# heracles-ec/heracles

Hardware: AMD Instinct MI355X
Metric: map->Cl pairs/sec + mixing-matrix build sec, nside=4096 lmax=6144 (higher is better)
Workload: dtype f64

## Files before the change

### heracles_amd/csrc/hx_analysis.hip

```cpp
#include <algorithm>
#include <cmath>
#include <cstdlib>
#include <cstring>

#include "hx_sht_common.h"

namespace hx {
using namespace hxfft;

constexpr int HALF_F = 1;
template <int SPIN>
struct LegCfg {
    static constexpr int NW = SPIN == 0 ? 16 : 8;
    static constexpr int NT = SPIN == 0 ? 1 : 2;
    static constexpr int NOP = SPIN == 0 ? 1 : 2;
    static constexpr int NPAR = (SPIN == 2 && HALF_F) ? 1 : 2;
};
int analysis_f_rows(int spin) { return spin == 0 ? LegCfg<0>::NPAR * LegCfg<0>::NOP : LegCfg<2>::NPAR * LegCfg<2>::NOP; }

struct LegParams {
    PlanDev P;
    const LegTask *__restrict__ tasks;
    const double *__restrict__ F;
    double *__restrict__ partial;
// ... 510 lines not shown
        if (l >= l0) {
            const int col = (c >> 3) * NCOL + 2 * (c & 7);
            for (int t = 0; t < mt.count; ++t) {
                const double *p = partial + (tasks[mt.first + t].pout - row0 + (l - l0)) * ncol + col;
                v.x += p[0];
                v.y += p[1];
            }
            if (fl) { v.x *= fl[l]; v.y *= fl[l]; }
        }
        double2 *dst = alm + (long long)c * alm_stride + almidx(lmax, l, m);
        if (add) { const double2 o = *dst; v.x += o.x; v.y += o.y; }
        *dst = v;
    }
}

static int ring_mlim(int lmax, int spin, double sth, double cth)
{
    double ofs = lmax * 0.01;
    if (ofs < 100.) ofs = 100.;
    double b = -2 * spin * fabs(cth);
    double t1 = lmax * sth + ofs;
    double c = (double)spin * spin - t1 * t1;
    double discr = b * b - 4 * c;
    if (discr <= 0) return lmax;
    double res = (-b + sqrt(discr)) / 2.;
    if (res > lmax) res = lmax;
    return (int)(res + 0.5);
}

struct SweepShape {
    int ng, nbx, valu, ncol, oneset, duo;
};
static SweepShape sweep_shape(int spin, int nb)
{
    const int cols = 2 * nb;
    SweepShape sh = {0, 0, 0, 0, 0, 0};
    if (cols <= 8) { sh.valu = 1; return sh; }
    sh.duo = 1;
    sh.oneset = spin == 2;
    sh.ng = std::max(cols / NCOL, 1);
    const int rem = cols > NCOL ? cols % NCOL : 0;
    const int maxbx = spin == 2 ? 2 : (sh.ng == 1 ? 1 : 0);
    if (rem > 4 * maxbx) sh.ng += 1;
// ... 147 lines not shown
    hx_plan::TaskSet &ts = blocks == 8 && blocks != valu_task_blocks(spin) ? (spin ? pl->ts[6] : pl->ts[7]) : (spin ? pl->ts[4] : pl->ts[5]);
    HX_TRY(build_task_set(pl, spin, blocks, ts));
    *out = &ts;
    return HX_OK;
}

int synth_duo_tasks(hx_plan *pl, int spin, hx_plan::TaskSet **out)
{
    if (spin) HX_TRY(ensure_rec2(pl));
    hx_plan::TaskSet &ts = spin ? pl->ts[3] : pl->ts[2];
    HX_TRY(build_task_set(pl, spin, PipeCfg<2>::NW * (spin ? PipeCfg<2>::RBS : PipeCfg<0>::RBS), ts));
    DevBuf &lim = spin ? pl->syn_mlim2 : pl->syn_mlim0;
    if (!lim.p) {
        std::vector<int> h(pl->nrp_pad, -1);
        for (int rp = 0; rp < pl->nrp; ++rp) {
            const int last = std::min(rp / RBLK * RBLK + RBLK - 1, pl->nrp - 1);
            h[rp] = std::min(pl->lmax, ring_mlim(pl->lmax, spin, pl->h_sth[last], pl->h_z[last]));
        }
        HX_TRY(upload(lim, h));
    }
    *out = &ts;
    return HX_OK;
}

static int analysis_batch_valu(hx_plan *pl, int spin, int nb, const double *d_maps, double2 *d_alms, const double *d_rw,
                               const double *d_pw, const double *d_fl, int add)
{
    hx_plan::TaskSet *tsp = nullptr;
    HX_TRY(valu_tasks(pl, spin, &tsp));
    hx_plan::TaskSet &ts = *tsp;
    if (pl->hsrc == nullptr && pl->nssrc == nullptr) {
        HX_TRY(pl->Y.alloc(sizeof(double2) * (size_t)pl->ny * nb));
        HX_TRY(launch_ring_subdft_maps(pl, nb, d_maps, d_pw, pl->Y.as<double2>()));
    }
    double budget = 80e9;
    if (scratch_budget_bytes() > 0.0) budget = scratch_budget_bytes();
    else {
        size_t fr = 0, tot = 0;
        if (hipMemGetInfo(&fr, &tot) == hipSuccess) budget = std::min(budget, 0.5 * (double)(fr + pl->F.bytes + pl->partial.bytes));
        budget = std::max(budget, 2e9);
    }
    const int lmax = pl->lmax, pcol = valu_partial_cols(spin), unit = spin ? 2 : 1;
    const double f_per_m = (double)pl->nrp_pad * valu_operand_doubles(spin) * sizeof(double);
    const std::vector<long long> &prow = ts.rows_before_m;
    std::vector<std::pair<int, int>> chunks;
    size_t maxF = 16, maxP = 16;
    const int m_end = pl->m_hi < 0 ? lmax + 1 : std::min(pl->m_hi, lmax + 1), ms = std::max(pl->m_step, 1);
    for (int m0 = std::max(pl->m_lo, 0); m0 < m_end;) {
// ... 31 lines not shown

int analysis_batch(hx_plan *pl, int spin, int nb, const double *d_maps, double2 *d_alms, const double *d_rw,
                   const double *d_pw, const double *d_fl, int add)
{
    if (valu_batch(spin, nb)) return analysis_batch_valu(pl, spin, nb, d_maps, d_alms, d_rw, d_pw, d_fl, add);
    const int sidx = spin ? 1 : 0;
    HX_TRY(build_tasks(pl, spin));
    if (spin) HX_TRY(ensure_rec2(pl));
    const SweepShape sh = sweep_shape(spin, nb);
    const bool one_set = sh.oneset || duo_shape(sh);
    if (one_set) HX_TRY(build_task_set(pl, spin, PipeCfg<2>::NW * (spin ? PipeCfg<2>::RBS : PipeCfg<0>::RBS), spin ? pl->ts[3] : pl->ts[2]));
    hx_plan::TaskSet &ts = one_set ? (spin ? pl->ts[3] : pl->ts[2]) : pl->ts[sidx];
    const int ncol = sh.ncol;
    if (pl->hsrc == nullptr && pl->nssrc == nullptr) {
        HX_TRY(pl->Y.alloc(sizeof(double2) * (size_t)pl->ny * nb));
        HX_TRY(launch_ring_subdft_maps(pl, nb, d_maps, d_pw, pl->Y.as<double2>()));
    }

    double budget = 80e9;
    if (scratch_budget_bytes() > 0.0) budget = scratch_budget_bytes();
    else {
        size_t fr = 0, tot = 0;
        if (hipMemGetInfo(&fr, &tot) == hipSuccess)
            budget = std::min(budget, 0.5 * (double)(fr + pl->F.bytes + pl->partial.bytes));
        budget = std::max(budget, 2e9);
    }
    const double f_per_m = (double)pl->nrp_pad * analysis_f_rows(spin) * ncol * sizeof(double);
    const int lmax = pl->lmax;
    const std::vector<long long> &prow = ts.arow;
    const int pcol = sweep_pcol(sh);
    std::vector<std::pair<int, int>> chunks;
// ... 99 lines not shown
    HX_HIP(hipMemsetAsync(pl->partial.p, 0, (size_t)stream_tasks(pl, s.spin).arow[pl->lmax + 1] * sweep_pcol(sh) * sizeof(double), rt().stream));
    pl->last_chunks = 1;
    return HX_OK;
}

template <int SPIN>
static int stream_slab(StreamSweep &s, int k)
{
    hx_plan *pl = s.pl;
    hx_plan::TaskSet &ts = stream_tasks(pl, SPIN);
    const SweepShape sh = sweep_shape(SPIN, s.nb);
    const int ng = sh.ng + (sh.nbx > 0 ? 1 : 0), lmax = pl->lmax, nm = lmax + 1;
    const int rp_lo = s.rp_edge[k], rp_hi = s.rp_edge[k + 1];
    hipStream_t st = rt().stream;
    PlanDev P = pl->dev();
    HX_TRY(launch_ring_subdft_maps(pl, s.nb, s.d_maps, s.d_pw, pl->Y.as<double2>(), rp_lo, std::min(rp_hi, pl->nrp)));
    {
        ProfScope ps("fourier_combine");
        const int tile_hi = k + 1 == s.nslab ? pl->nrp_pad / 32 : rp_hi / 32;
        dim3 grid(nm, tile_hi - rp_lo / 32);
        hipLaunchKernelGGL(k_fourier_combine<SPIN>, grid, dim3(256), 0, st, P, pl->Y.as<double2>(), s.nb, ng, sh.ncol, 0, 1, s.d_rw,
                           ts.d_tasks.as<LegTask>(), ts.d_of_m.as<MTasks>(), pl->F.as<double>(), rp_lo / 32);
    }
    {
        ProfScope ps("legendre_analysis");
        ProfScope ps2(SPIN == 0 ? "legendre_analysis_s0" : "legendre_analysis_s2");
        LegParams A;
        A.P = P; A.tasks = ts.d_tasks.as<LegTask>(); A.F = pl->F.as<double>(); A.partial = pl->partial.as<double>();
        A.m0 = 0; A.ms = 1; A.row0 = 0; A.ng = ng; A.ncol = sh.ncol; A.pcol = sweep_pcol(sh);
        A.of_m = s.d_of_m.as<MTasks>() + (size_t)k * (lmax + 1); A.arow = ts.d_arow.as<long long>(); A.arow0 = 0; A.add_all = 1;
        HX_TRY(launch_duo<SPIN>(sh, dim3((unsigned)nm), st, A, SPIN == 0 ? pl->cn0.as<double2>() : pl->cn2.as<double2>()));
// ... 90 lines not shown
```

### heracles_amd/csrc/hx_fft_core.h

```cpp
#pragma once
#ifdef __HIPCC__
#include <hip/hip_runtime.h>
#define HX_HD __host__ __device__ __forceinline__
#else
#include <cmath>
#define HX_HD inline
struct double2 {
    double x, y;
};
#endif

namespace hxfft {

HX_HD double2 mk(double a, double b)
{
    double2 r;
    r.x = a;
    r.y = b;
    return r;
}
HX_HD double2 cadd(double2 a, double2 b) { return mk(a.x + b.x, a.y + b.y); }
HX_HD double2 csub(double2 a, double2 b) { return mk(a.x - b.x, a.y - b.y); }
HX_HD double2 cmul(double2 a, double2 b) { return mk(a.x * b.x - a.y * b.y, a.x * b.y + a.y * b.x); }
HX_HD double2 cmulc(double2 a, double2 b)
// ... 16 lines not shown
}

HX_HD int ilog2(unsigned v)
{
    int p = 0;
    while ((1u << p) < v) ++p;
    return p;
}

HX_HD int fft_size_for(int n)
{
    if ((n & (n - 1)) == 0) return n;
    int m = 1;
    while (m < 2 * n - 1) m <<= 1;
    return m;
}

struct TwFactored {
    const double2 *hi, *lo;
    HX_HD double2 operator[](int k) const
    {
        const double2 a = hi[k >> 6], b = lo[k & 63];
        double2 r;
        r.x = a.x * b.x - a.y * b.y;
        r.y = a.x * b.y + a.y * b.x;
        return r;
    }
};

HX_HD int lds_slot(int e) { return e + (e >> 4) + (e >> 9); }
// ... 159 lines not shown
```

### heracles_amd/csrc/hx_legendre_valu.hip

```cpp
#include <algorithm>
#include <cmath>

#include "hx_sht_common.h"

namespace hx {
using namespace hxfft;

constexpr int VALU_R0 = 8;
constexpr int VALU_R2 = 6;
constexpr int VALU_LB0 = 8;
constexpr int VALU_LB2 = 4;
template <int SPIN>
struct ValuCfg {
    static constexpr int R = SPIN == 0 ? VALU_R0 : VALU_R2;
    static constexpr int LB = SPIN == 0 ? VALU_LB0 : VALU_LB2;
    static constexpr int NA = SPIN == 0 ? 2 : 4;
    static constexpr int NF = SPIN == 0 ? 4 : 8;
    static constexpr int NRB = 2 * R;
    static_assert(LB * NA == 32 || LB * NA == 16, "the butterfly below reduces 16 or 32 accumulators");
};

int valu_task_blocks(int spin) { return spin == 0 ? ValuCfg<0>::NRB : ValuCfg<2>::NRB; }
int valu_partial_cols(int spin) { return spin == 0 ? ValuCfg<0>::NA : ValuCfg<2>::NA; }
int valu_operand_doubles(int spin) { return spin == 0 ? ValuCfg<0>::NF : ValuCfg<2>::NF; }
// ... 5 lines not shown
    const LegTask *__restrict__ tasks;
    const double *__restrict__ F;
    double *__restrict__ partial;
    int m0, ms;
    long long row0;
};

template <int SPIN>
__global__ __launch_bounds__(256) void k_fourier_combine_valu(PlanDev P, const double2 *__restrict__ Y, int c0, int m0, int ms,
                                                              const double *__restrict__ rw, const LegTask *__restrict__ tasks,
                                                              const MTasks *__restrict__ of_m, double *__restrict__ F)
{
    constexpr int NF = ValuCfg<SPIN>::NF;
    const int m = m0 + blockIdx.x * ms;
    const MTasks mt = of_m[m];
    if (mt.count == 0 || ((int)blockIdx.y + 1) * 256 <= tasks[mt.first].rb0 * RBLK) return;
    const int rp = blockIdx.y * 256 + threadIdx.x;
    if (rp >= P.nrp_pad) return;
    double *row = F + ((long long)blockIdx.x * P.nrp_pad + rp) * NF;
    double o[NF];
#pragma unroll
    for (int k = 0; k < NF; ++k) o[k] = 0.0;
    if (rp < P.nrp) {
        const RingAtM ram = ring_at_m_of(P, rp, m, rw);
        if (SPIN == 0) {
            double2 fn, fs;
            ring_modes_ns(P, Y, c0, rp, m, ram, fn, fs);
            o[0] = fn.x + fs.x; o[1] = fn.y + fs.y;
            o[2] = fn.x - fs.x; o[3] = fn.y - fs.y;
        } else {
            double2 qn, qs, un, us;
            ring_modes_ns(P, Y, c0, rp, m, ram, qn, qs);
// ... 626 lines not shown
```

### heracles_amd/csrc/hx_sht.hip

```cpp
#include <algorithm>
#include <chrono>
#include <cmath>
#include <cstdlib>

#include <type_traits>

#include "hx_sht_common.h"


namespace hx {
using namespace hxfft;

__global__ void k_init_norm0(int lmax, double2 *__restrict__ coef, double *__restrict__ alpha)
{
    const int t = blockIdx.x * blockDim.x + threadIdx.x;
    const int m = t >> 1, par = t & 1;
    if (m > lmax) return;
    const double dm = m;
    auto a = [dm](double l) { return sqrt((4.0 * l * l - 1.0) / (l * l - dm * dm)); };
    double al = 1.0;
    for (int l = m + par; l <= lmax; l += 2) {
        const double dl = l;
        const double a1 = a(dl + 1.0), a2 = a(dl + 2.0);
        const double A = a1 * a2;
// ... 23 lines not shown
        const double r1 = sqrt((2.0 * k + 3.0) / (2.0 * k + 1.0));
        const double p = r1 * (2.0 * k + 1.0) * k * lp / den;
        const double q = -r1 * (2.0 * k + 1.0) * dm * dn / den;
        double a1 = 1.0;
        if (l > l0) {
            const double r2 = sqrt((2.0 * k + 3.0) / (2.0 * k - 1.0));
            const double r = r2 * lp * sqrt((k * k - dm * dm) * (k * k - dn * dn)) / den;
            a1 = r * am1;
        }
        coef[almidx(lmax, l + 1, m)] = make_double2(p * a0 / a1, q * a0 / a1);
        am1 = a0;
        a0 = a1;
    }
}

__global__ __launch_bounds__(512) void k_init_bhat(PlanDev P, const int *__restrict__ rp_list,
                                                   double2 *__restrict__ bhat)
{
    extern __shared__ double2 buf[];
    const int rp = rp_list[blockIdx.x];
    const int n = P.nsub[rp];
    const int M = fft_size_for(n);
    for (int j = threadIdx.x; j < lds_fft_slots(M); j += blockDim.x) buf[j] = make_double2(0.0, 0.0);
    __syncthreads();
    for (int j = threadIdx.x; j < n; j += blockDim.x) {
        double2 c = expipi((double)chirp_num(j, n) / (double)n);
        buf[lds_slot(j)] = c;
        if (j) buf[lds_slot(M - j)] = c;
    }
    __syncthreads();
    lds_fft_dif(buf, M, P.tw, P.twN);
    double2 *out = bhat + P.bhat_off[rp];
    for (int e = threadIdx.x; e < M; e += blockDim.x) out[M >= 16 ? (e & 15) * (M >> 4) + (e >> 4) : e] = buf[lds_slot(e)];
}

__host__ __device__ inline int ring_ph_hi(int M) { return (4 * M) / 64 + 1; }
constexpr int RING_NTMAX = 512;
constexpr int RING_FB = 8;

template <int MODE, bool WSYM = false>
__global__ __launch_bounds__(RING_NTMAX) void k_ring_subdft(PlanDev P, const RingDesc *__restrict__ desc, int nrings, int nb, int Mclass,
                                                            const double *__restrict__ maps,
                                                            const double *__restrict__ pixw,
                                                            const double2 *__restrict__ zin,
                                                            double2 *__restrict__ Y, double *__restrict__ pixout = nullptr,
                                                            const double *__restrict__ ref = nullptr)
{
// ... 6 lines not shown
    int tid = threadIdx.x;
    auto ring_of = [&](int item) __attribute__((always_inline)) { return ((item >> 5) / nb) * 8 + (item & 7); };
    RingDesc cur = RingDesc{0, 0, 0, 1, 0};
    if ((int)blockIdx.x < nitems && ring_of(blockIdx.x) < nrings) cur = desc[ring_of(blockIdx.x)];
    for (int item = blockIdx.x; item < nitems; item += gridDim.x) {
        const int r = (item >> 3) & 3, set = item >> 5;
        const int ring = ring_of(item), c = set % nb;
        const int itn = item + gridDim.x, ringn = itn < nitems ? ring_of(itn) : nrings;
        const bool nextv = ringn < nrings;
        if (ring >= nrings) {
            if (nextv) cur = desc[ringn];
            continue;
        }
        const int n = cur.n;
        const long long sN = cur.sN, sS = cur.sS;
        const int M = fft_size_for(n), MP = lds_fft_slots(M);
        const bool blu = M != n;
        const int p = ilog2(M);
        const double2 *bh = P.bhat + cur.bhat_off;
        const double inv = 1.0 / M, inv4n = 0.25 / (double)n;
        asm volatile("; item" : "+v"(tid));
        const bool haveS = sS >= 0, odd = r & 1, pw = MODE == 0 && !WSYM && pixw != nullptr;
        constexpr bool wsym = MODE == 0 && WSYM;
        const double sg = (r & 2) ? -1.0 : 1.0;
        const double *mpN = maps + (long long)c * P.npix + sN, *mpS = maps + (long long)c * P.npix + (haveS ? sS : sN);
        const double *pwN = pixw + sN, *pwS = pixw + (haveS ? sS : sN);
        const double2 *zp = zin + (long long)c * P.ny + sN;
        double2 z[RING_FB][4];
        struct __attribute__((aligned(8))) Pair { double x, y; };
        Pair wsy[RING_FB / 2];
        auto load_batch_t = [&](auto WIDEC, int u0) __attribute__((always_inline)) {
            constexpr bool WIDE = decltype(WIDEC)::value;
// ... 86 lines not shown
                }
                u0 += RING_FB;
                if (u0 * nt >= n) break;
                load_batch(u0);
            }
            if (blu)
                for (int j = n + tid; j < M; j += nt) buf[lds_slot(j)] = make_double2(0.0, 0.0);
        }
        __syncthreads();
        if (nextv) {
            auto sc = [](int v) __attribute__((always_inline)) { return __builtin_amdgcn_readfirstlane(v); };
            cur.sN = ((long long)sc(nd0.y) << 32) | (unsigned)sc(nd0.x);
            cur.sS = ((long long)sc(nd0.w) << 32) | (unsigned)sc(nd0.z);
            cur.bhat_off = ((long long)sc(nd1.y) << 32) | (unsigned)sc(nd1.x);
            cur.n = sc(nd1.z);
            cur.rp = sc(nd1.w);
        }
        double2 *out = Y + (long long)c * P.ny + sN + (long long)r * n;
        double *pxN = nullptr, *pxS = nullptr;
        const double *rfN = nullptr, *rfS = nullptr;
        if (MODE == 1 && pixout) {
            pxN = pixout + (long long)c * P.npix + sN + r;
            pxS = pixout + (long long)c * P.npix + (haveS ? sS : sN) + r;
            if (ref) { rfN = ref + (long long)c * P.npix + sN + r; rfS = ref + (long long)c * P.npix + (haveS ? sS : sN) + r; }
        }
        const int kdrop0 = MODE == 0 ? (P.lmax - r) / 4 + 1 : n, kdrop1 = (4 * n - P.lmax - r + 3) / 4;
        auto emit = [&](int k, double2 v) __attribute__((always_inline)) {
            if (MODE == 0 && k >= kdrop0 && k < kdrop1) return;
            if (MODE == 1 && pxN) {
                double fn = v.x, fs = -v.y;
                if (rfN) { fn = rfN[4 * k] - fn; fs = rfS[4 * k] - fs; }
                pxN[4 * k] = fn;
                if (haveS) pxS[4 * k] = fs;
            } else {
                out[k] = v;
            }
        };
        if (!blu) {
            lds_fft_dif(buf, M, twf, P.twN);
            for (int k = tid; k < n; k += nt) emit(k, buf[lds_slot(bitrev(k, p))]);
            continue;
// ... 18 lines not shown
#pragma unroll
                    for (int j = 0; j < 16; ++j) bq[j] = bh[j * nbf + i + nt];
                }
                dit_inv_regs<4>(x);
#pragma unroll
                for (int j = 0; j < 16; ++j) buf[lds_slot(16 * i) + j] = x[j];
            }
            __syncthreads();
            lds_fft_dit_inv(buf, M, twf, P.twN, tid, nt, true);
        } else {
            lds_fft_dif(buf, M, twf, P.twN, tid, nt);
            for (int j = tid; j < M; j += nt) buf[lds_slot(j)] = cmul(buf[lds_slot(j)], bh[j]);
            __syncthreads();
            lds_fft_dit_inv(buf, M, twf, P.twN, tid, nt);
        }
        for (int k = tid; k < n; k += nt)
            emit(k, cscale(cmul(buf[lds_slot(k)], phase(2u * mod_by_inv((unsigned)k * (unsigned)k, 2u * (unsigned)n, 2.0 * inv4n))), inv));
    }
}

template <int MODE, bool WSYM = false>
__global__ __launch_bounds__(RING_NTMAX) void k_ring_pairfft(PlanDev P, const RingDesc *__restrict__ desc, int nrings, int nb, int M,
                                                             const double *__restrict__ maps, const double *__restrict__ pixw,
                                                             const double2 *__restrict__ zin, double2 *__restrict__ Y,
                                                             double *__restrict__ pixout = nullptr, const double *__restrict__ ref = nullptr)
{
    extern __shared__ double2 buf[];
    __shared__ double2 tw_hi[TW_HI_MAX], tw_lo[64];
    const int MP = lds_fft_slots(M), n = M, p = ilog2(M);
    double2 *ph_hi = buf + 2 * MP, *ph_lo = ph_hi + ring_ph_hi(M);
    const int nt = blockDim.x, nh = nt >> 1;
    const int nitems = ((nrings + 7) >> 3) * nb * 16;
// ... 58 lines not shown
    };
    using H0 = std::integral_constant<int, 0>;
    using H1 = std::integral_constant<int, RING_FB / 2>;
    bool have_half = false;
    for (int item = blockIdx.x; item < nitems; item += gridDim.x) {
        const int rpair = (item >> 3) & 1;
        const int ring = ring_of(item), c = comp_of(item);
        const int itn = item + gridDim.x, ringn = itn < nitems ? ring_of(itn) : nrings;
        const bool nextv = ringn < nrings;
        if (ring >= nrings) {
            if (nextv) cur = desc[ringn];
            have_half = false;
            continue;
        }
        const long long sN = cur.sN, sS = cur.sS;
        asm volatile("; item" : "+v"(tid));
        const bool haveS = sS >= 0;
        if (!have_half) request(H0{}, cur, c);
        request(H1{}, cur, c);
        int4 nd0 = make_int4(0, 0, 0, 0);
        if (nextv) nd0 = *(reinterpret_cast<const int4 *>(desc + ringn) + (tid >> 30));
        {
        __builtin_amdgcn_s_waitcnt(0xc07f);
        __builtin_amdgcn_s_barrier();
        finish(haveS);
#pragma unroll
        for (int u = 0; u < RING_FB; ++u) {
            const int j = 2 * (tid + (u >> 1) * nt) + (u & 1);
            if (j >= n) continue;
            const double2 e0 = rpair ? csub(z[u][0], z[u][2]) : cadd(z[u][0], z[u][2]);
            const double2 e1 = rpair ? mul_mi(csub(z[u][1], z[u][3])) : cadd(z[u][1], z[u][3]);
            const double2 t0 = cadd(e0, e1);
            buf[lds_slot(j)] = rpair ? cmul(t0, phase((unsigned)j)) : t0;
            buf[MP + lds_slot(j)] = cmul(csub(e0, e1), phase((unsigned)j * (unsigned)(rpair + 2)));
        }
        __syncthreads();
        have_half = false;
        if (nextv) {
            cur.sN = ((long long)__builtin_amdgcn_readfirstlane(nd0.y) << 32) | (unsigned)__builtin_amdgcn_readfirstlane(nd0.x);
            cur.sS = ((long long)__builtin_amdgcn_readfirstlane(nd0.w) << 32) | (unsigned)__builtin_amdgcn_readfirstlane(nd0.z);
            request(H0{}, cur, comp_of(itn));
            have_half = true;
        }
        const int half = tid >= nh ? 1 : 0, gt = tid - half * nh;
        double2 *bh = buf + half * MP;
        lds_fft_dif(bh, M, twf, P.twN, gt, nh);
        const int r = rpair + 2 * half;
        if (MODE == 1 && pixout) {
            double *pxN = pixout + (long long)c * P.npix + sN + r, *pxS = pixout + (long long)c * P.npix + (haveS ? sS : sN) + r;
            if (ref) {
                const double *rfN = ref + (long long)c * P.npix + sN + r, *rfS = ref + (long long)c * P.npix + (haveS ? sS : sN) + r;
                for (int k = gt; k < n; k += nh) {
                    const double2 v = bh[lds_slot(bitrev(k, p))];
                    pxN[4 * k] = rfN[4 * k] - v.x;
                    if (haveS) pxS[4 * k] = rfS[4 * k] + v.y;
                }
            } else {
                for (int k = gt; k < n; k += nh) {
                    const double2 v = bh[lds_slot(bitrev(k, p))];
                    pxN[4 * k] = v.x;
                    if (haveS) pxS[4 * k] = -v.y;
                }
            }
        } else {
            double2 *out = Y + (long long)c * P.ny + sN + (long long)r * n;
            const int kdrop0 = MODE == 0 ? (P.lmax - r) / 4 + 1 : n, kdrop1 = (4 * n - P.lmax - r + 3) / 4;
            for (int k = gt; k < n; k += nh)
                if (k < kdrop0 || k >= kdrop1) *(out + k) = bh[lds_slot(bitrev(k, p))];
        }
        }
    }
}

constexpr int SPLIT_JMAX = 16;

__global__ __launch_bounds__(512) void k_init_bhat_split(PlanDev P, const int *__restrict__ rp_list, int C,
                                                          double2 *__restrict__ bhat)
{
    extern __shared__ double2 buf[];
    const int rp = rp_list[blockIdx.x];
    const int n = P.nsub[rp], M = 2 * C;
// ... 6 lines not shown
        __syncthreads();
        for (int j = threadIdx.x; j < C; j += blockDim.x) {
            const double2 b0 = b_at(j), b1 = b_at(j + C);
            buf[lds_slot(j)] = half == 0 ? cadd(b0, b1) : cmul(csub(b0, b1), P.tw[j]);
        }
        __syncthreads();
        lds_fft_dif(buf, C, P.tw, P.twN);
        for (int j = threadIdx.x; j < C; j += blockDim.x) out[half * C + j] = buf[lds_slot(j)];
    }
}

template <int MODE>
__global__ __launch_bounds__(512) void k_ring_subdft_split(PlanDev P, const int *__restrict__ rp_list, int C,
                                                            const double *__restrict__ maps, const double *__restrict__ pixw,
                                                            const double2 *__restrict__ zin, double2 *__restrict__ Y,
                                                            double *__restrict__ pixout = nullptr, const double *__restrict__ ref = nullptr)
{
    extern __shared__ double2 buf[];
    const int rp = rp_list[blockIdx.y];
    const int c = blockIdx.z;
    const int n = P.nsub[rp];
    const long long sN = P.startN[rp], sS = P.startS[rp];
    const int M = 2 * C;
    const bool plain = fft_size_for(n) == n;
    const double *mp = maps + (long long)c * P.npix;
    const double2 *zp = zin + (long long)c * P.ny + sN;
    const double2 *bh = P.bhat + (plain ? 0 : P.bhat_off[rp]);
    const double inv = 1.0 / M;
    __shared__ double2 tw_hi[TW_HI_MAX], tw_lo[64];
    const TwFactored twf = load_tw_factored(tw_hi, tw_lo, P.tw, P.twN);
    auto z_at = [&](int j, int q) {
        if (MODE == 0) {
            const long long iN = sN + j + (long long)q * n;
            double fn = mp[iN];
            if (pixw) fn *= pixw[iN];
            double fs = 0.0;
            if (sS >= 0) {
                const long long iS = sS + j + (long long)q * n;
                fs = mp[iS];
                if (pixw) fs *= pixw[iS];
            }
            return make_double2(fn, fs);
        }
        return zp[j + (long long)q * n];
    };
    auto emit = [&](int r, int k, double2 v, bool add) __attribute__((always_inline)) {
        if (MODE == 1 && pixout) {
            const long long iN = (long long)c * P.npix + sN + 4 * k + r, iS = (long long)c * P.npix + sS + 4 * k + r;
            if (add) {
                pixout[iN] += ref ? -v.x : v.x;
                if (sS >= 0) pixout[iS] += ref ? v.y : -v.y;
            } else {
                double fn = v.x, fs = -v.y;
                if (ref) { fn = ref[iN] - fn; if (sS >= 0) fs = ref[iS] - fs; }
                pixout[iN] = fn;
                if (sS >= 0) pixout[iS] = fs;
            }
        } else {
            double2 *o = Y + (long long)c * P.ny + sN + (long long)r * n + k;
            *o = add ? cadd(*o, v) : v;
        }
// ... 238 lines not shown
            sth[rp] = sqrt((1.0 - z[rp]) * (1.0 + z[rp]));
            nsub[rp] = nside; sN[rp] = ncap + (long long)(i - nside) * 4 * ns;
            shifted[rp] = ((i - nside) & 1) == 0;
        }
        sS[rp] = i == 2 * nside ? -1 : pl->npix - sN[rp] - 4LL * nsub[rp];
        maxM = std::max(maxM, fft_size_for(nsub[rp]));
    }
    pl->ny = sN[pl->nrp - 1] + 4LL * nsub[pl->nrp - 1];
    const int cap = lds_fft_cap();
    if (maxM > 2 * cap || (maxM > cap && nside > 0 && [&] { for (int rp = 0; rp < pl->nrp; ++rp) if (fft_size_for(nsub[rp]) > cap && fft_size_for(nsub[rp]) == nsub[rp]) return true; return false; }())) {
        set_error("hx_plan_create: nside=%d needs an in-LDS FFT of %d points (limit %d, %d for Bluestein rings); unsupported", nside, maxM, cap, 2 * cap);
        delete pl;
        return nullptr;
    }
    pl->fft_cap = cap;
    {
        std::map<std::pair<int, int>, std::vector<int>> byM;
        for (int rp = pl->nrp - 1; rp >= 0; --rp) {
            const int M = fft_size_for(nsub[rp]);
            const bool pair = M == nsub[rp] && M >= 16 && M <= cap && (2 * (size_t)lds_fft_slots(M) + ring_ph_hi(M) + 64) * sizeof(double2) + 4096 <= 160 * 1024;
            byM[{M, pair ? -1 : 0}].push_back(rp);
        }
        std::vector<int> list;
        for (auto it = byM.rbegin(); it != byM.rend(); ++it) {
            hx_plan::FftClass c;
            c.M = it->first.first; c.big = it->first.second; c.first = (int)list.size(); c.count = (int)it->second.size();
            list.insert(list.end(), it->second.begin(), it->second.end());
            pl->fft_classes.push_back(c);
        }
        if (upload(pl->fft_rp_list, list) != HX_OK) { delete pl; return nullptr; }
        pl->h_fft_rp_list = list;
    }
    pl->twN = std::max(maxM, 2);
    pl->lds_fft = (size_t)lds_fft_slots(std::min(maxM, cap)) * sizeof(double2);
    pl->h_sth = sth; pl->h_z = z; pl->h_nsub = nsub; pl->h_startN = sN; pl->h_startS = sS;
    std::vector<int> blu_list, blu_split;
    long long btot = 0;
    {
        std::map<int, long long> off_of_n;
        for (int rp = 0; rp < pl->nrp; ++rp) {
            int n = nsub[rp], M = fft_size_for(n);
            if (M == n) continue;
            auto it = off_of_n.find(n);
            if (it == off_of_n.end()) {
                it = off_of_n.emplace(n, btot).first;
                btot += M;
                (M > cap ? blu_split : blu_list).push_back(rp);
            }
            boff[rp] = it->second;
        }
    }
    int rc = HX_OK;
    auto chk = [&](int r) { if (rc == HX_OK) rc = r; };
    chk(upload(pl->z, z)); chk(upload(pl->omz, omz)); chk(upload(pl->sth, sth)); chk(upload(pl->rwdef, rw));
    chk(upload(pl->nsub, nsub)); chk(upload(pl->shifted, shifted));
    chk(upload(pl->startN, sN)); chk(upload(pl->startS, sS)); chk(upload(pl->bhat_off, boff));
    {
        std::vector<RingDesc> desc(pl->h_fft_rp_list.size());
        for (size_t k = 0; k < desc.size(); ++k) {
            const int rp = pl->h_fft_rp_list[k];
            desc[k] = RingDesc{sN[rp], sS[rp], boff[rp], nsub[rp], rp};
        }
        chk(upload(pl->fft_desc, desc));
    }
    chk(pl->bhat.alloc(sizeof(double2) * std::max<long long>(btot, 1)));
    if (rc != HX_OK || plan_tables(pl) != HX_OK) { delete pl; return nullptr; }
    hipStream_t st = rt().stream;
    if (!blu_list.empty()) {
        DevBuf d_list;
        if (upload(d_list, blu_list) != HX_OK) { delete pl; return nullptr; }
        hipLaunchKernelGGL(k_init_bhat, dim3((unsigned)blu_list.size()), dim3(512), pl->lds_fft, st, pl->dev(),
                           d_list.as<int>(), pl->bhat.as<double2>());
        (void)hipStreamSynchronize(st);
    }
    if (!blu_split.empty()) {
        DevBuf d_list;
        if (upload(d_list, blu_split) != HX_OK) { delete pl; return nullptr; }
        hipLaunchKernelGGL(k_init_bhat_split, dim3((unsigned)blu_split.size()), dim3(std::min(512, std::max(64, cap / 16))), (size_t)lds_fft_slots(cap) * sizeof(double2), st,
                           pl->dev(), d_list.as<int>(), cap, pl->bhat.as<double2>());
        (void)hipStreamSynchronize(st);
    }
    if (hipStreamSynchronize(st) != hipSuccess || hipGetLastError() != hipSuccess) {
        set_error("hx_plan_create: table initialisation failed");
        delete pl;
        return nullptr;
    }
    return pl;
// ... 68 lines not shown
namespace hx {
int ensure_rec2(hx_plan *pl)
{
    if (pl->cn2.p) return HX_OK;
    HX_TRY(pl->cn2.alloc(sizeof(double2) * (pl->nlm + TABLE_PAD)));
    HX_TRY(pl->al2.alloc(sizeof(double) * (pl->nlm + TABLE_PAD)));
    HX_HIP(hipMemsetAsync(pl->cn2.p, 0, sizeof(double2) * (pl->nlm + TABLE_PAD), rt().stream));
    HX_HIP(hipMemsetAsync(pl->al2.p, 0, sizeof(double) * (pl->nlm + TABLE_PAD), rt().stream));
    hipLaunchKernelGGL(k_init_norm2, dim3((pl->lmax + 64) / 64), dim3(64), 0, rt().stream, pl->lmax, pl->cn2.as<double2>(), pl->al2.as<double>());
    HX_HIP(hipGetLastError());
    return HX_OK;
}

template <int MODE>
static int launch_subdft_classes(hx_plan *pl, int nb, const double *d_maps, const double *d_pw, const double2 *zin, double2 *Y, int rp_lo = 0,
                                 int rp_hi = 0x7fffffff, double *pixout = nullptr, const double *ref = nullptr)
{
    for (const auto &cls : pl->fft_classes) {
        hx_plan::FftClass c = cls;
        if (rp_lo > 0 || rp_hi < pl->nrp) {
            const int *b = pl->h_fft_rp_list.data() + cls.first, *e = b + cls.count;
            const int *x = std::lower_bound(b, e, rp_hi, [](int rp, int lim) { return rp >= lim; });
            const int *y = std::lower_bound(b, e, rp_lo, [](int rp, int lim) { return rp >= lim; });
            c.first = cls.first + (int)(x - b);
            c.count = (int)(y - x);
            if (c.count <= 0) continue;
        }
        if (c.big < 0) {
            const int threads = 2 * std::max(64, c.M / 16);
            const size_t lds = (size_t)(2 * lds_fft_slots(c.M) + ring_ph_hi(c.M) + 64) * sizeof(double2);
            const int per_cu = (int)std::max<size_t>(1, std::min<size_t>(512 / threads, (160 * 1024) / (lds + 3 * 1024 + 256)));
            const long long items = ((long long)c.count + 7) / 8 * nb * 16;
            const unsigned groups = (unsigned)std::min<long long>(items, (long long)rt().cus * per_cu);
            if (MODE == 0 && d_pw && pl->pw_mode == 2) {
                hipLaunchKernelGGL((k_ring_pairfft<MODE, MODE == 0>), dim3(groups), dim3(threads), lds, rt().stream,
                                   pl->dev(), pl->fft_desc.as<RingDesc>() + c.first, c.count, nb, c.M, d_maps, d_pw, zin, Y, pixout, ref);
            } else {
                hipLaunchKernelGGL((k_ring_pairfft<MODE, false>), dim3(groups), dim3(threads), lds, rt().stream,
                                   pl->dev(), pl->fft_desc.as<RingDesc>() + c.first, c.count, nb, c.M, d_maps, d_pw, zin, Y, pixout, ref);
            }
            continue;
        }
        if (c.M > pl->fft_cap || c.big) {
            const int C = std::min(c.M, pl->fft_cap), threads = std::min(512, std::max(64, C / SPLIT_JMAX));
            hipLaunchKernelGGL(k_ring_subdft_split<MODE>, dim3(1, c.count, nb), dim3(threads), (size_t)lds_fft_slots(C) * sizeof(double2), rt().stream,
                               pl->dev(), pl->fft_rp_list.as<int>() + c.first, C, d_maps, d_pw, zin, Y, pixout, ref);
            continue;
        }
        const int threads = std::min(RING_NTMAX, std::max(64, c.M / 16));
        const size_t lds = (size_t)(lds_fft_slots(c.M) + ring_ph_hi(c.M) + 64) * sizeof(double2);
        const int per_cu = (int)std::max<size_t>(1, std::min<size_t>(512 / threads, (160 * 1024) / (lds + 3 * 1024 + 256)));
        const long long items = ((long long)c.count + 7) / 8 * nb * 32;
        const unsigned groups = (unsigned)std::min<long long>(items, (long long)rt().cus * per_cu);
        if (MODE == 0 && d_pw && pl->pw_mode == 2) {
            hipLaunchKernelGGL((k_ring_subdft<MODE, MODE == 0>), dim3(groups), dim3(threads), lds, rt().stream,
                               pl->dev(), pl->fft_desc.as<RingDesc>() + c.first, c.count, nb, c.M, d_maps, d_pw, zin, Y, pixout, ref);
        } else {
            hipLaunchKernelGGL((k_ring_subdft<MODE, false>), dim3(groups), dim3(threads), lds, rt().stream,
                               pl->dev(), pl->fft_desc.as<RingDesc>() + c.first, c.count, nb, c.M, d_maps, d_pw, zin, Y, pixout, ref);
        }
    }
    HX_HIP(hipGetLastError());
    return HX_OK;
}

__global__ __launch_bounds__(256) void k_pixw_symmetry(PlanDev P, const double *__restrict__ pixw, int *__restrict__ flag)
{
    const int rp = blockIdx.x, n = P.nsub[rp];
    const long long sN = P.startN[rp], sS = P.startS[rp];
    bool ok = true;
    for (int j = threadIdx.x; j < n; j += blockDim.x) {
        const double w = pixw[sN + j];
#pragma unroll
        for (int q = 1; q < 4; ++q) ok = ok && pixw[sN + j + (long long)q * n] == w;
        if (sS >= 0) {
#pragma unroll
            for (int q = 0; q < 4; ++q) ok = ok && pixw[sS + j + (long long)q * n] == w;
        }
    }
    if (!ok) *flag = 0;
}

int launch_ring_subdft_maps(hx_plan *pl, int nb, const double *d_maps, const double *d_pw, double2 *Y, int rp_lo, int rp_hi)
{
    ProfScope ps("ring_fft");
    if (d_pw && pl->pw_checked != d_pw) HX_TRY(classify_pixel_weights(pl, d_pw));
    return launch_subdft_classes<0>(pl, nb, d_maps, d_pw, nullptr, Y, rp_lo, rp_hi);
}

int classify_pixel_weights(hx_plan *pl, const double *d_pw)
{
    pl->pw_checked = d_pw;
    pl->pw_mode = 0;
    if (!d_pw || pl->nside < 1) return HX_OK;
    HX_TRY(pl->pw_sym.alloc(sizeof(int)));
    HX_HIP(hipMemsetAsync(pl->pw_sym.p, 1, sizeof(int), rt().stream));
    hipLaunchKernelGGL(k_pixw_symmetry, dim3(pl->nrp), dim3(256), 0, rt().stream, pl->dev(), d_pw, pl->pw_sym.as<int>());
    int flag = 0;
    HX_HIP(hipMemcpyAsync(&flag, pl->pw_sym.p, sizeof(int), hipMemcpyDeviceToHost, rt().stream));
    HX_HIP(hipStreamSynchronize(rt().stream));
    pl->pw_mode = flag != 0 ? 2 : 1;
    return HX_OK;
// ... 419 lines not shown
```

### heracles_amd/csrc/hx_sht_common.h

```cpp
#pragma once
#include <map>
#include <vector>

#include "hx_common.h"
#include "hx_fft_core.h"

namespace hx {

typedef double double4_t __attribute__((ext_vector_type(4)));

constexpr int LBLK = 32;
constexpr int NCOL = 16;
constexpr int TABLE_PAD = 512;
constexpr int NGMAX = 2;
constexpr int RBLK = 32;
constexpr double SC_BIG = 0x1p+300, SC_SMALL = 0x1p-300;

struct LegTask {
    int m;
    int rb0;
    int nrb;
    int pad;
    long long pout;
};

struct MTasks {
    int first, count;
};

struct alignas(16) RingDesc {
    long long sN, sS, bhat_off;
    int n, rp;
};
struct PlanDev {
    int nside, lmax, nrp, nrp_pad, twN;
    long long npix, ny;
    const double *z, *omz, *sth, *rwdef;
    const int *nsub, *shifted;
    const long long *startN, *startS, *bhat_off;
    const double2 *tw, *bhat;
    const double *mfac, *kfac2;
    const double2 *rec0;
    const double4 *rec2;
    double wnorm;
    const double2 *hsrc;
    long long hsrc_stride;
    int hN;
// ... 246 lines not shown
    std::vector<int> h_nsub;
    std::vector<long long> h_startN, h_startS;
    struct TaskSet {
        bool built = false;
        std::vector<hx::LegTask> tasks;
        std::vector<hx::MTasks> of_m;
        std::vector<long long> rows_before_m;
        std::vector<long long> arow;
        hx::DevBuf d_tasks, d_of_m, d_arow;
    } ts[8];
    struct FftClass { int M, first, count, big; };
    std::vector<FftClass> fft_classes;
    hx::DevBuf fft_rp_list;
    hx::DevBuf fft_desc;
    std::vector<int> h_fft_rp_list;
    hx::DevBuf Y, F, partial, d_dbg, resid_maps, pw_sym;
    hx::DevBuf syn_mlim0, syn_mlim2;
    hx::DevBuf syn_tab, syn_boff0, syn_boff2;
    const double *pw_checked = nullptr;
    int pw_mode = 0;
    static constexpr int NSTAGE = 3;
    hx::DevBuf stage[NSTAGE];
    hipEvent_t stage_done[NSTAGE] = {nullptr, nullptr, nullptr};
    static constexpr int NUNIT_EV = 4;
    hipEvent_t unit_up[NUNIT_EV] = {nullptr, nullptr, nullptr, nullptr};
    hx::PlanDev dev() const;
};

namespace hx {
hx_plan *plan_create_equiangular(int N, int lmax);
int ensure_rec2(hx_plan *pl);
int launch_ring_subdft_maps(hx_plan *pl, int nb, const double *d_maps, const double *d_pw, double2 *Y, int rp_lo = 0, int rp_hi = 0x7fffffff);
int classify_pixel_weights(hx_plan *pl, const double *d_pw);
int build_tasks(hx_plan *pl, int spin);
int analysis_batch(hx_plan *pl, int spin, int nb, const double *d_maps, double2 *d_alms, const double *d_rw,
                   const double *d_pw, const double *d_fl, int add);
int analysis_max_comp(int spin);
int analysis_next_batch(int spin, int remaining);
int analysis_max_batch(int spin, int ncomp);
struct StreamSweep {
    hx_plan *pl = nullptr;
    int spin = 0, nb = 0, nslab = 0;
    const double *d_maps = nullptr, *d_rw = nullptr, *d_pw = nullptr, *d_fl = nullptr;
    double2 *d_alms = nullptr;
    std::vector<int> rp_edge;
    DevBuf d_of_m;
};
// ... 21 lines not shown
```

Baseline: 424.4.

## Prune Bluestein ring FFTs to per-ring m-limit in analysis

Computes a per-ring maximum useful order (the same m-limit used by the Legendre sweep, max of spin 0 and 2) and builds a second set of FFT classes whose Bluestein convolution size only needs to cover that order. This gives smaller padded FFTs, with their own chirp tables, for polar rings. Coefficients above the limit are dropped at emit time, and the VALU Legendre kernel's early-exit check moves from block level to thread level. The cost is extra plan-time tables and bhat memory, plus correctness risk from reading the negative frequencies out of the pruned circular convolution.

```diff
diff --git a/heracles_amd/csrc/hx_analysis.hip b/heracles_amd/csrc/hx_analysis.hip
--- a/heracles_amd/csrc/hx_analysis.hip
+++ b/heracles_amd/csrc/hx_analysis.hip
@@ -548,19 +548,6 @@
     }
 }
 
-static int ring_mlim(int lmax, int spin, double sth, double cth)
-{
-    double ofs = lmax * 0.01;
-    if (ofs < 100.) ofs = 100.;
-    double b = -2 * spin * fabs(cth);
-    double t1 = lmax * sth + ofs;
-    double c = (double)spin * spin - t1 * t1;
-    double discr = b * b - 4 * c;
-    if (discr <= 0) return lmax;
-    double res = (-b + sqrt(discr)) / 2.;
-    if (res > lmax) res = lmax;
-    return (int)(res + 0.5);
-}
 
 struct SweepShape {
     int ng, nbx, valu, ncol, oneset, duo;
@@ -738,8 +725,7 @@
     if (!lim.p) {
         std::vector<int> h(pl->nrp_pad, -1);
         for (int rp = 0; rp < pl->nrp; ++rp) {
-            const int last = std::min(rp / RBLK * RBLK + RBLK - 1, pl->nrp - 1);
-            h[rp] = std::min(pl->lmax, ring_mlim(pl->lmax, spin, pl->h_sth[last], pl->h_z[last]));
+            h[rp] = ring_block_mlim(pl->lmax, spin, pl->h_sth.data(), pl->h_z.data(), pl->nrp, RBLK, rp);
         }
         HX_TRY(upload(lim, h));
     }
@@ -755,7 +741,7 @@
     hx_plan::TaskSet &ts = *tsp;
     if (pl->hsrc == nullptr && pl->nssrc == nullptr) {
         HX_TRY(pl->Y.alloc(sizeof(double2) * (size_t)pl->ny * nb));
-        HX_TRY(launch_ring_subdft_maps(pl, nb, d_maps, d_pw, pl->Y.as<double2>()));
+        HX_TRY(launch_ring_subdft_maps(pl, nb, d_maps, d_pw, pl->Y.as<double2>(), 0, 0x7fffffff, true));
     }
     double budget = 80e9;
     if (scratch_budget_bytes() > 0.0) budget = scratch_budget_bytes();
@@ -817,7 +803,7 @@
     const int ncol = sh.ncol;
     if (pl->hsrc == nullptr && pl->nssrc == nullptr) {
         HX_TRY(pl->Y.alloc(sizeof(double2) * (size_t)pl->ny * nb));
-        HX_TRY(launch_ring_subdft_maps(pl, nb, d_maps, d_pw, pl->Y.as<double2>()));
+        HX_TRY(launch_ring_subdft_maps(pl, nb, d_maps, d_pw, pl->Y.as<double2>(), 0, 0x7fffffff, true));
     }
 
     double budget = 80e9;
@@ -947,7 +933,7 @@
     const int rp_lo = s.rp_edge[k], rp_hi = s.rp_edge[k + 1];
     hipStream_t st = rt().stream;
     PlanDev P = pl->dev();
-    HX_TRY(launch_ring_subdft_maps(pl, s.nb, s.d_maps, s.d_pw, pl->Y.as<double2>(), rp_lo, std::min(rp_hi, pl->nrp)));
+    HX_TRY(launch_ring_subdft_maps(pl, s.nb, s.d_maps, s.d_pw, pl->Y.as<double2>(), rp_lo, std::min(rp_hi, pl->nrp), true));
     {
         ProfScope ps("fourier_combine");
         const int tile_hi = k + 1 == s.nslab ? pl->nrp_pad / 32 : rp_hi / 32;
diff --git a/heracles_amd/csrc/hx_fft_core.h b/heracles_amd/csrc/hx_fft_core.h
--- a/heracles_amd/csrc/hx_fft_core.h
+++ b/heracles_amd/csrc/hx_fft_core.h
@@ -54,6 +54,37 @@
     int m = 1;
     while (m < 2 * n - 1) m <<= 1;
     return m;
+}
+
+HX_HD int ring_mlim(int lmax, int spin, double sth, double cth)
+{
+    double ofs = lmax * 0.01;
+    if (ofs < 100.) ofs = 100.;
+    double b = -2 * spin * fabs(cth);
+    double t1 = lmax * sth + ofs;
+    double c = (double)spin * spin - t1 * t1;
+    double discr = b * b - 4 * c;
+    if (discr <= 0) return lmax;
+    double res = (-b + sqrt(discr)) / 2.;
+    if (res > lmax) res = lmax;
+    return (int)(res + 0.5);
+}
+HX_HD int ring_block_mlim(int lmax, int spin, const double *sth, const double *cth, int nrp, int rblk, int rp)
+{
+    int last = rp / rblk * rblk + rblk - 1;
+    if (last > nrp - 1) last = nrp - 1;
+    const int l = ring_mlim(lmax, spin, sth[last], cth[last]);
+    return l < lmax ? l : lmax;
+}
+HX_HD int fft_lim_k2(int L) { return L / 4 + 1; }
+HX_HD int fft_size_lim(int n, int L)
+{
+    const int M0 = fft_size_for(n);
+    if (M0 == n || L < 0) return M0;
+    const int need = n + 2 * fft_lim_k2(L) + 1;
+    int m = 1;
+    while (m < need) m <<= 1;
+    return m < M0 ? m : M0;
 }
 
 struct TwFactored {
diff --git a/heracles_amd/csrc/hx_legendre_valu.hip b/heracles_amd/csrc/hx_legendre_valu.hip
--- a/heracles_amd/csrc/hx_legendre_valu.hip
+++ b/heracles_amd/csrc/hx_legendre_valu.hip
@@ -43,8 +43,8 @@
     constexpr int NF = ValuCfg<SPIN>::NF;
     const int m = m0 + blockIdx.x * ms;
     const MTasks mt = of_m[m];
-    if (mt.count == 0 || ((int)blockIdx.y + 1) * 256 <= tasks[mt.first].rb0 * RBLK) return;
     const int rp = blockIdx.y * 256 + threadIdx.x;
+    if (mt.count == 0 || rp < tasks[mt.first].rb0 * RBLK) return;
     if (rp >= P.nrp_pad) return;
     double *row = F + ((long long)blockIdx.x * P.nrp_pad + rp) * NF;
     double o[NF];
diff --git a/heracles_amd/csrc/hx_sht.hip b/heracles_amd/csrc/hx_sht.hip
--- a/heracles_amd/csrc/hx_sht.hip
+++ b/heracles_amd/csrc/hx_sht.hip
@@ -61,23 +61,21 @@
     }
 }
 
-__global__ __launch_bounds__(512) void k_init_bhat(PlanDev P, const int *__restrict__ rp_list,
-                                                   double2 *__restrict__ bhat)
+__global__ __launch_bounds__(512) void k_init_bhat(PlanDev P, const BhatSpec *__restrict__ specs, double2 *__restrict__ bhat)
 {
     extern __shared__ double2 buf[];
-    const int rp = rp_list[blockIdx.x];
-    const int n = P.nsub[rp];
-    const int M = fft_size_for(n);
+    const BhatSpec sp = specs[blockIdx.x];
+    const int n = sp.n, M = sp.M;
     for (int j = threadIdx.x; j < lds_fft_slots(M); j += blockDim.x) buf[j] = make_double2(0.0, 0.0);
     __syncthreads();
-    for (int j = threadIdx.x; j < n; j += blockDim.x) {
+    for (int j = threadIdx.x; j <= max(sp.lo, sp.hi); j += blockDim.x) {
         double2 c = expipi((double)chirp_num(j, n) / (double)n);
-        buf[lds_slot(j)] = c;
-        if (j) buf[lds_slot(M - j)] = c;
+        if (j <= sp.hi) buf[lds_slot(j)] = c;
+        if (j && j <= sp.lo) buf[lds_slot(M - j)] = c;
     }
     __syncthreads();
     lds_fft_dif(buf, M, P.tw, P.twN);
-    double2 *out = bhat + P.bhat_off[rp];
+    double2 *out = bhat + sp.off;
     for (int e = threadIdx.x; e < M; e += blockDim.x) out[M >= 16 ? (e & 15) * (M >> 4) + (e >> 4) : e] = buf[lds_slot(e)];
 }
 
@@ -114,8 +112,9 @@
         }
         const int n = cur.n;
         const long long sN = cur.sN, sS = cur.sS;
-        const int M = fft_size_for(n), MP = lds_fft_slots(M);
-        const bool blu = M != n;
+        const int M = MODE == 0 ? Mclass : fft_size_for(n), MP = lds_fft_slots(M);
+        const bool blu = M != n, pruned = MODE == 0 && blu && M < 2 * n - 1;
+        const int Lr = min(P.lmax, cur.mlim);
         const int p = ilog2(M);
         const double2 *bh = P.bhat + cur.bhat_off;
         const double inv = 1.0 / M, inv4n = 0.25 / (double)n;
@@ -232,7 +231,7 @@
             cur.sS = ((long long)sc(nd0.w) << 32) | (unsigned)sc(nd0.z);
             cur.bhat_off = ((long long)sc(nd1.y) << 32) | (unsigned)sc(nd1.x);
             cur.n = sc(nd1.z);
-            cur.rp = sc(nd1.w);
+            cur.mlim = sc(nd1.w);
         }
         double2 *out = Y + (long long)c * P.ny + sN + (long long)r * n;
         double *pxN = nullptr, *pxS = nullptr;
@@ -242,7 +241,7 @@
             pxS = pixout + (long long)c * P.npix + (haveS ? sS : sN) + r;
             if (ref) { rfN = ref + (long long)c * P.npix + sN + r; rfS = ref + (long long)c * P.npix + (haveS ? sS : sN) + r; }
         }
-        const int kdrop0 = MODE == 0 ? (P.lmax - r) / 4 + 1 : n, kdrop1 = (4 * n - P.lmax - r + 3) / 4;
+        const int kdrop0 = MODE == 0 ? (Lr - r) / 4 + 1 : n, kdrop1 = (4 * n - Lr - r + 3) / 4;
         auto emit = [&](int k, double2 v) __attribute__((always_inline)) {
             if (MODE == 0 && k >= kdrop0 && k < kdrop1) return;
             if (MODE == 1 && pxN) {
@@ -291,8 +290,12 @@
             __syncthreads();
             lds_fft_dit_inv(buf, M, twf, P.twN, tid, nt);
         }
-        for (int k = tid; k < n; k += nt)
-            emit(k, cscale(cmul(buf[lds_slot(k)], phase(2u * mod_by_inv((unsigned)k * (unsigned)k, 2u * (unsigned)n, 2.0 * inv4n))), inv));
+        for (int k = tid; k < n; k += nt) {
+            if (MODE == 0 && k >= kdrop0 && k < kdrop1) continue;
+            const bool neg = pruned && k >= kdrop1;
+            const int kk = neg ? n - k : k;
+            emit(k, cscale(cmul(buf[lds_slot(neg ? M - kk : k)], phase(2u * mod_by_inv((unsigned)kk * (unsigned)kk, 2u * (unsigned)n, 2.0 * inv4n))), inv));
+        }
     }
 }
 
@@ -381,12 +384,17 @@
             continue;
         }
         const long long sN = cur.sN, sS = cur.sS;
+        const int Lr = min(P.lmax, cur.mlim);
         asm volatile("; item" : "+v"(tid));
         const bool haveS = sS >= 0;
         if (!have_half) request(H0{}, cur, c);
         request(H1{}, cur, c);
         int4 nd0 = make_int4(0, 0, 0, 0);
-        if (nextv) nd0 = *(reinterpret_cast<const int4 *>(desc + ringn) + (tid >> 30));
+        int ndl = 0;
+        if (nextv) {
+            nd0 = *(reinterpret_cast<const int4 *>(desc + ringn) + (tid >> 30));
+            ndl = *(reinterpret_cast<const int *>(desc + ringn) + 7 + (tid >> 30));
+        }
         {
         __builtin_amdgcn_s_waitcnt(0xc07f);
         __builtin_amdgcn_s_barrier();
@@ -406,6 +414,7 @@
         if (nextv) {
             cur.sN = ((long long)__builtin_amdgcn_readfirstlane(nd0.y) << 32) | (unsigned)__builtin_amdgcn_readfirstlane(nd0.x);
             cur.sS = ((long long)__builtin_amdgcn_readfirstlane(nd0.w) << 32) | (unsigned)__builtin_amdgcn_readfirstlane(nd0.z);
+            cur.mlim = __builtin_amdgcn_readfirstlane(ndl);
             request(H0{}, cur, comp_of(itn));
             have_half = true;
         }
@@ -431,7 +440,7 @@
             }
         } else {
             double2 *out = Y + (long long)c * P.ny + sN + (long long)r * n;
-            const int kdrop0 = MODE == 0 ? (P.lmax - r) / 4 + 1 : n, kdrop1 = (4 * n - P.lmax - r + 3) / 4;
+            const int kdrop0 = MODE == 0 ? (Lr - r) / 4 + 1 : n, kdrop1 = (4 * n - Lr - r + 3) / 4;
             for (int k = gt; k < n; k += nh)
                 if (k < kdrop0 || k >= kdrop1) *(out + k) = bh[lds_slot(bitrev(k, p))];
         }
@@ -468,12 +477,14 @@
 __global__ __launch_bounds__(512) void k_ring_subdft_split(PlanDev P, const int *__restrict__ rp_list, int C,
                                                             const double *__restrict__ maps, const double *__restrict__ pixw,
                                                             const double2 *__restrict__ zin, double2 *__restrict__ Y,
-                                                            double *__restrict__ pixout = nullptr, const double *__restrict__ ref = nullptr)
+                                                            double *__restrict__ pixout = nullptr, const double *__restrict__ ref = nullptr,
+                                                            const int *__restrict__ mlim = nullptr)
 {
     extern __shared__ double2 buf[];
     const int rp = rp_list[blockIdx.y];
     const int c = blockIdx.z;
     const int n = P.nsub[rp];
+    const int Lr = MODE == 0 && mlim ? min(P.lmax, mlim[rp]) : 4 * n;
     const long long sN = P.startN[rp], sS = P.startS[rp];
     const int M = 2 * C;
     const bool plain = fft_size_for(n) == n;
@@ -499,6 +510,7 @@
         return zp[j + (long long)q * n];
     };
     auto emit = [&](int r, int k, double2 v, bool add) __attribute__((always_inline)) {
+        if (MODE == 0 && k >= (Lr - r) / 4 + 1 && k < (4 * n - Lr - r + 3) / 4) return;
         if (MODE == 1 && pixout) {
             const long long iN = (long long)c * P.npix + sN + 4 * k + r, iS = (long long)c * P.npix + sS + 4 * k + r;
             if (add) {
@@ -767,27 +779,36 @@
         return nullptr;
     }
     pl->fft_cap = cap;
-    {
+    std::vector<int> alim(pl->nrp);
+    for (int rp = 0; rp < pl->nrp; ++rp)
+        alim[rp] = std::max(ring_block_mlim(lmax, 0, sth.data(), z.data(), pl->nrp, RBLK, rp), ring_block_mlim(lmax, 2, sth.data(), z.data(), pl->nrp, RBLK, rp));
+    pl->h_ana_mlim = alim;
+    auto build_classes = [&](bool lim, std::vector<hx_plan::FftClass> &classes, std::vector<int> &list) {
         std::map<std::pair<int, int>, std::vector<int>> byM;
         for (int rp = pl->nrp - 1; rp >= 0; --rp) {
-            const int M = fft_size_for(nsub[rp]);
+            const int M = lim ? fft_size_lim(nsub[rp], alim[rp]) : fft_size_for(nsub[rp]);
             const bool pair = M == nsub[rp] && M >= 16 && M <= cap && (2 * (size_t)lds_fft_slots(M) + ring_ph_hi(M) + 64) * sizeof(double2) + 4096 <= 160 * 1024;
             byM[{M, pair ? -1 : 0}].push_back(rp);
         }
-        std::vector<int> list;
         for (auto it = byM.rbegin(); it != byM.rend(); ++it) {
             hx_plan::FftClass c;
             c.M = it->first.first; c.big = it->first.second; c.first = (int)list.size(); c.count = (int)it->second.size();
             list.insert(list.end(), it->second.begin(), it->second.end());
-            pl->fft_classes.push_back(c);
-        }
-        if (upload(pl->fft_rp_list, list) != HX_OK) { delete pl; return nullptr; }
-        pl->h_fft_rp_list = list;
+            classes.push_back(c);
+        }
+    };
+    build_classes(false, pl->fft_classes, pl->h_fft_rp_list);
+    build_classes(true, pl->fft_classes_lim, pl->h_fft_rp_list_lim);
+    if (upload(pl->fft_rp_list, pl->h_fft_rp_list) != HX_OK || upload(pl->fft_rp_list_lim, pl->h_fft_rp_list_lim) != HX_OK || upload(pl->ana_mlim, alim) != HX_OK) {
+        delete pl;
+        return nullptr;
     }
     pl->twN = std::max(maxM, 2);
     pl->lds_fft = (size_t)lds_fft_slots(std::min(maxM, cap)) * sizeof(double2);
     pl->h_sth = sth; pl->h_z = z; pl->h_nsub = nsub; pl->h_startN = sN; pl->h_startS = sS;
-    std::vector<int> blu_list, blu_split;
+    std::vector<int> blu_split;
+    std::vector<BhatSpec> blu_list;
+    std::vector<long long> boff_lim(pl->nrp, -1);
     long long btot = 0;
     {
         std::map<int, long long> off_of_n;
@@ -797,10 +818,25 @@
             auto it = off_of_n.find(n);
             if (it == off_of_n.end()) {
                 it = off_of_n.emplace(n, btot).first;
+                if (M > cap) blu_split.push_back(rp);
+                else blu_list.push_back(BhatSpec{btot, n, M, n - 1, n - 1});
                 btot += M;
-                (M > cap ? blu_split : blu_list).push_back(rp);
             }
             boff[rp] = it->second;
+        }
+        std::map<std::pair<int, int>, long long> off_of_nl;
+        for (int rp = 0; rp < pl->nrp; ++rp) {
+            const int n = nsub[rp], M = fft_size_lim(n, alim[rp]);
+            boff_lim[rp] = boff[rp];
+            if (M == fft_size_for(n)) continue;
+            auto it = off_of_nl.find({n, alim[rp]});
+            if (it == off_of_nl.end()) {
+                it = off_of_nl.emplace(std::make_pair(n, alim[rp]), btot).first;
+                const int K2 = fft_lim_k2(alim[rp]);
+                blu_list.push_back(BhatSpec{btot, n, M, n - 1 + K2, K2});
+                btot += M;
+            }
+            boff_lim[rp] = it->second;
         }
     }
     int rc = HX_OK;
@@ -812,9 +848,14 @@
         std::vector<RingDesc> desc(pl->h_fft_rp_list.size());
         for (size_t k = 0; k < desc.size(); ++k) {
             const int rp = pl->h_fft_rp_list[k];
-            desc[k] = RingDesc{sN[rp], sS[rp], boff[rp], nsub[rp], rp};
+            desc[k] = RingDesc{sN[rp], sS[rp], boff[rp], nsub[rp], lmax};
         }
         chk(upload(pl->fft_desc, desc));
+        for (size_t k = 0; k < desc.size(); ++k) {
+            const int rp = pl->h_fft_rp_list_lim[k];
+            desc[k] = RingDesc{sN[rp], sS[rp], boff_lim[rp], nsub[rp], alim[rp]};
+        }
+        chk(upload(pl->fft_desc_lim, desc));
     }
     chk(pl->bhat.alloc(sizeof(double2) * std::max<long long>(btot, 1)));
     if (rc != HX_OK || plan_tables(pl) != HX_OK) { delete pl; return nullptr; }
@@ -823,7 +864,7 @@
         DevBuf d_list;
         if (upload(d_list, blu_list) != HX_OK) { delete pl; return nullptr; }
         hipLaunchKernelGGL(k_init_bhat, dim3((unsigned)blu_list.size()), dim3(512), pl->lds_fft, st, pl->dev(),
-                           d_list.as<int>(), pl->bhat.as<double2>());
+                           d_list.as<BhatSpec>(), pl->bhat.as<double2>());
         (void)hipStreamSynchronize(st);
     }
     if (!blu_split.empty()) {
@@ -922,12 +963,15 @@
 
 template <int MODE>
 static int launch_subdft_classes(hx_plan *pl, int nb, const double *d_maps, const double *d_pw, const double2 *zin, double2 *Y, int rp_lo = 0,
-                                 int rp_hi = 0x7fffffff, double *pixout = nullptr, const double *ref = nullptr)
-{
-    for (const auto &cls : pl->fft_classes) {
+                                 int rp_hi = 0x7fffffff, double *pixout = nullptr, const double *ref = nullptr, bool order_limit = false)
+{
+    const bool lim = MODE == 0 && order_limit;
+    const std::vector<int> &h_list = lim ? pl->h_fft_rp_list_lim : pl->h_fft_rp_list;
+    const RingDesc *descs = (lim ? pl->fft_desc_lim : pl->fft_desc).as<RingDesc>();
+    for (const auto &cls : lim ? pl->fft_classes_lim : pl->fft_classes) {
         hx_plan::FftClass c = cls;
         if (rp_lo > 0 || rp_hi < pl->nrp) {
-            const int *b = pl->h_fft_rp_list.data() + cls.first, *e = b + cls.count;
+            const int *b = h_list.data() + cls.first, *e = b + cls.count;
             const int *x = std::lower_bound(b, e, rp_hi, [](int rp, int lim) { return rp >= lim; });
             const int *y = std::lower_bound(b, e, rp_lo, [](int rp, int lim) { return rp >= lim; });
             c.first = cls.first + (int)(x - b);
@@ -942,17 +986,18 @@
             const unsigned groups = (unsigned)std::min<long long>(items, (long long)rt().cus * per_cu);
             if (MODE == 0 && d_pw && pl->pw_mode == 2) {
                 hipLaunchKernelGGL((k_ring_pairfft<MODE, MODE == 0>), dim3(groups), dim3(threads), lds, rt().stream,
-                                   pl->dev(), pl->fft_desc.as<RingDesc>() + c.first, c.count, nb, c.M, d_maps, d_pw, zin, Y, pixout, ref);
+                                   pl->dev(), descs + c.first, c.count, nb, c.M, d_maps, d_pw, zin, Y, pixout, ref);
             } else {
                 hipLaunchKernelGGL((k_ring_pairfft<MODE, false>), dim3(groups), dim3(threads), lds, rt().stream,
-                                   pl->dev(), pl->fft_desc.as<RingDesc>() + c.first, c.count, nb, c.M, d_maps, d_pw, zin, Y, pixout, ref);
+                                   pl->dev(), descs + c.first, c.count, nb, c.M, d_maps, d_pw, zin, Y, pixout, ref);
             }
             continue;
         }
         if (c.M > pl->fft_cap || c.big) {
             const int C = std::min(c.M, pl->fft_cap), threads = std::min(512, std::max(64, C / SPLIT_JMAX));
             hipLaunchKernelGGL(k_ring_subdft_split<MODE>, dim3(1, c.count, nb), dim3(threads), (size_t)lds_fft_slots(C) * sizeof(double2), rt().stream,
-                               pl->dev(), pl->fft_rp_list.as<int>() + c.first, C, d_maps, d_pw, zin, Y, pixout, ref);
+                               pl->dev(), (lim ? pl->fft_rp_list_lim : pl->fft_rp_list).as<int>() + c.first, C, d_maps, d_pw, zin, Y, pixout, ref,
+                               lim ? pl->ana_mlim.as<int>() : (const int *)nullptr);
             continue;
         }
         const int threads = std::min(RING_NTMAX, std::max(64, c.M / 16));
@@ -962,10 +1007,10 @@
         const unsigned groups = (unsigned)std::min<long long>(items, (long long)rt().cus * per_cu);
         if (MODE == 0 && d_pw && pl->pw_mode == 2) {
             hipLaunchKernelGGL((k_ring_subdft<MODE, MODE == 0>), dim3(groups), dim3(threads), lds, rt().stream,
-                               pl->dev(), pl->fft_desc.as<RingDesc>() + c.first, c.count, nb, c.M, d_maps, d_pw, zin, Y, pixout, ref);
+                               pl->dev(), descs + c.first, c.count, nb, c.M, d_maps, d_pw, zin, Y, pixout, ref);
         } else {
             hipLaunchKernelGGL((k_ring_subdft<MODE, false>), dim3(groups), dim3(threads), lds, rt().stream,
-                               pl->dev(), pl->fft_desc.as<RingDesc>() + c.first, c.count, nb, c.M, d_maps, d_pw, zin, Y, pixout, ref);
+                               pl->dev(), descs + c.first, c.count, nb, c.M, d_maps, d_pw, zin, Y, pixout, ref);
         }
     }
     HX_HIP(hipGetLastError());
@@ -989,11 +1034,11 @@
     if (!ok) *flag = 0;
 }
 
-int launch_ring_subdft_maps(hx_plan *pl, int nb, const double *d_maps, const double *d_pw, double2 *Y, int rp_lo, int rp_hi)
+int launch_ring_subdft_maps(hx_plan *pl, int nb, const double *d_maps, const double *d_pw, double2 *Y, int rp_lo, int rp_hi, bool order_limit)
 {
     ProfScope ps("ring_fft");
     if (d_pw && pl->pw_checked != d_pw) HX_TRY(classify_pixel_weights(pl, d_pw));
-    return launch_subdft_classes<0>(pl, nb, d_maps, d_pw, nullptr, Y, rp_lo, rp_hi);
+    return launch_subdft_classes<0>(pl, nb, d_maps, d_pw, nullptr, Y, rp_lo, rp_hi, nullptr, nullptr, order_limit);
 }
 
 int classify_pixel_weights(hx_plan *pl, const double *d_pw)
diff --git a/heracles_amd/csrc/hx_sht_common.h b/heracles_amd/csrc/hx_sht_common.h
--- a/heracles_amd/csrc/hx_sht_common.h
+++ b/heracles_amd/csrc/hx_sht_common.h
@@ -30,7 +30,12 @@
 
 struct alignas(16) RingDesc {
     long long sN, sS, bhat_off;
-    int n, rp;
+    int n;
+    int mlim;
+};
+struct BhatSpec {
+    long long off;
+    int n, M, lo, hi;
 };
 struct PlanDev {
     int nside, lmax, nrp, nrp_pad, twN;
@@ -307,6 +312,9 @@
     hx::DevBuf fft_rp_list;
     hx::DevBuf fft_desc;
     std::vector<int> h_fft_rp_list;
+    std::vector<FftClass> fft_classes_lim;
+    hx::DevBuf fft_rp_list_lim, fft_desc_lim, ana_mlim;
+    std::vector<int> h_fft_rp_list_lim, h_ana_mlim;
     hx::DevBuf Y, F, partial, d_dbg, resid_maps, pw_sym;
     hx::DevBuf syn_mlim0, syn_mlim2;
     hx::DevBuf syn_tab, syn_boff0, syn_boff2;
@@ -323,7 +331,8 @@
 namespace hx {
 hx_plan *plan_create_equiangular(int N, int lmax);
 int ensure_rec2(hx_plan *pl);
-int launch_ring_subdft_maps(hx_plan *pl, int nb, const double *d_maps, const double *d_pw, double2 *Y, int rp_lo = 0, int rp_hi = 0x7fffffff);
+int launch_ring_subdft_maps(hx_plan *pl, int nb, const double *d_maps, const double *d_pw, double2 *Y, int rp_lo = 0, int rp_hi = 0x7fffffff,
+                            bool order_limit = false);
 int classify_pixel_weights(hx_plan *pl, const double *d_pw);
 int build_tasks(hx_plan *pl, int spin);
 int analysis_batch(hx_plan *pl, int spin, int nb, const double *d_maps, double2 *d_alms, const double *d_rw,
```

Result: no change. 428.2 (median of 6 runs) (+0.9%).
